# timescale/pgvectorscale

Measured on AMD Instinct MI355X. Metric: QPS at recall@10>=0.99, higher is better.
Workload: dtype u64 xor+popcount (SBQ) / f32 (rerank)

## Files before the change

pgvectorscale_amd/csrc/vs_batch.hip:

```cpp
#include <thread>
#include <cstdarg>
#include <cmath>
#include <algorithm>
#include <cstdlib>

#include <atomic>
#include <mutex>
#include <unordered_map>

#include "vs_internal.h"


static uint32_t knob_u32(const char* name, int tuned, uint32_t dflt) {
    const char* v = vs_opt_get(name);
    if (v && *v) return (uint32_t)strtoul(v, nullptr, 10);
    return tuned >= 0 ? (uint32_t)tuned : dflt;
}

static uint32_t gload_pct() { return std::min<uint32_t>(std::max<uint32_t>(env_u32("VS_F_GLOAD_PCT", 75), 25), 90); }

static Caps initial_caps(const vs_index* ix, uint32_t L, uint32_t M) {
    uint64_t visits = 2ull * L + M + 32;
    uint64_t pushes = visits * ix->d.num_neighbors;
    Caps c;
// ... 281 lines not shown
    return v && *v;
}
static uint32_t visited_want(uint32_t L) { return (uint32_t)std::min<uint64_t>((uint64_t)L + L / 2 + 32, 1u << 20); }

static int candidate_holds(vs_index* ix, const FastLaunch& base, const FastLaunch& cand, uint64_t num, uint64_t den, bool* holds,
                           const char* base_name = nullptr, const char* cand_name = nullptr, const char* tail = "") {
    uint32_t res_base = 0, res_cand = 0;
    VS_TRY(fast_resident_scans(ix, base, &res_base));
    VS_TRY(fast_resident_scans(ix, cand, &res_cand));
    if (base_name && env_u32("VS_WS_DEBUG", 0))
        fprintf(stderr, "[VS_WS_DEBUG] resident scans: %s %u, %s %u%s\n", base_name, res_base, cand_name, res_cand, tail);
    *holds = num * res_cand >= den * res_base;
    return VS_OK;
}

static int choose_table_bitmap(vs_index* ix, FastLaunch& f, uint32_t vmode, bool phase, bool* slot_eligible) {
    *slot_eligible = false;
    if (f.lh != 0 || f.vr || !vmode || phase || f.gcap > (1u << 16)) return VS_OK;
    f.vwords = (f.gcap + 127) / 128;
    if (vmode < 2 || f.rc || f.gcap % 32 != 0) return VS_OK;
    *slot_eligible = true;
    FastLaunch g = f;
    g.vwords = f.gcap / 32;
    g.vslot = 1;
    bool holds = false;
    VS_TRY(candidate_holds(ix, f, g, 1, 1, &holds));
    if (holds || env_u32("VS_F_SLOTMAP_FORCE", 0)) f = g;
    return VS_OK;
}

static int choose_tables16(vs_index* ix, FastLaunch& f, uint32_t vmode, bool slot_eligible, bool keyed, uint32_t* gregion) {
    if (vmode != 3 || !f.vwords || !slot_eligible || f.lh != 0) return VS_OK;
    FastLaunch g = f;
    g.gcap = std::max<uint32_t>(next_pow2_u32(f.gcap), 1024);
    if (!fast_tables16_geometry(ix, g)) return VS_OK;
    g.glimit = (uint32_t)((uint64_t)g.gcap * gload_pct() / 100) - 64u;
    char tail[48];
    snprintf(tail, sizeof tail, "; gcap %u -> %u", f.gcap, g.gcap);
    bool holds = false;
    VS_TRY(candidate_holds(ix, f, g, keyed ? 3 : 5, keyed ? 2 : 4, &holds, "4-byte tables", "16-bit tables", tail));
    if (holds || env_u32("VS_F_SLOTMAP_FORCE", 0)) {
        f = g;
        *gregion = g.gregion;
    }
    return VS_OK;
}

static int choose_heap_top(vs_index* ix, FastLaunch& f, Caps& caps, bool phase) {
    if (f.lh != 0 || f.vr || f.hl != 511 || f.hcap <= 511 || phase || opt_is_set("VS_F_HL")) return VS_OK;
    FastLaunch h = f;
    h.hl = 255;
    h.gstride = round_up_u32(h.hcap - h.hl + 2, 2);
    bool holds = false;
    VS_TRY(candidate_holds(ix, f, h, 10, 11, &holds, "heap top 511", "255"));
    if (holds) {
        f = h;
        caps.f_hl = h.hl;
        caps.f_gstride = h.gstride;
    }
    return VS_OK;
}

static int choose_visited_ring(vs_index* ix, FastLaunch& f, uint32_t L, bool phase) {
    if (f.lh != 0 || f.vr || f.minw == 7 || phase) return VS_OK;
    const uint32_t want_v = visited_want(L);
    const uint32_t lean_v = round_up_u32(std::max<uint32_t>(want_v + 2 * want_v / 5, 64), 64);
    if (opt_is_set("VS_F_VCAP") || lean_v >= f.vcap) return VS_OK;
// ... 136 lines not shown
static int bind_timeline_buffer(vs_index* ix, FastLaunch& f, std::string* path) {
    const char* const tl_opt = vs_opt_get("VS_TIMELINE");
    *path = tl_opt ? tl_opt : "";
    if (path->empty()) return VS_OK;
    SearchWorkspace& w = ix->ws;
    VS_TRY(devbuf_reserve(ix->ctx, w.timeline, (size_t)f.nq * 16));
    VS_HIP(hipMemsetAsync(w.timeline.p, 0, (size_t)f.nq * 16, ix->ctx->stream));
    f.timeline = (uint64_t*)w.timeline.p;
    return VS_OK;
}
static int dump_timeline(vs_index* ix, uint32_t nq, const std::string& path) {
    std::vector<uint64_t> tl((size_t)nq * 2);
    VS_HIP(hipMemcpyAsync(tl.data(), ix->ws.timeline.p, tl.size() * 8, hipMemcpyDeviceToHost, ix->ctx->stream));
    VS_HIP(hipStreamSynchronize(ix->ctx->stream));
    if (FILE* fp = fopen(path.c_str(), "wb")) {
        fwrite(tl.data(), 8, tl.size(), fp);
        fclose(fp);
    }
    return VS_OK;
}

static int dump_fast_status(vs_index* ix, const FastLaunch& f, double pool_frac) {
    vs_ctx* c = ix->ctx;
    SearchWorkspace& w = ix->ws;
    std::vector<uint32_t> stv(f.nq);
    VS_HIP(hipMemcpyAsync(stv.data(), w.status.p, (size_t)f.nq * 4, hipMemcpyDeviceToHost, c->stream));
    uint32_t ctr[2] = {0, 0};
    VS_HIP(hipMemcpyAsync(ctr, w.pool_ctr.p, 4, hipMemcpyDeviceToHost, c->stream));
    VS_HIP(hipStreamSynchronize(c->stream));
    uint32_t hist[16] = {0};
    for (uint32_t v : stv) hist[v & 15]++;
    fprintf(stderr, "[VS_DEBUG_STATUS] fast kernel: lh=%u gcap=%u vr=%u minw=%u bitmap_words=%u (per %s); pool claims=%u of %u;",
            f.lh, f.gcap, f.vr, f.minw, f.vwords, f.vslot == 2 ? "slot, 16-bit entries" : f.vslot ? "slot" : "bucket", ctr[0], fast_pool_slots(f.nq, pool_frac));
    for (int i = 0; i < 16; ++i)
        if (hist[i]) fprintf(stderr, " status[%d]=%u", i, hist[i]);
    fprintf(stderr, "\n");
    return VS_OK;
}

static int run_fast_attempts(vs_index* ix, const BatchPlan& bp, Caps& caps, const int16_t* d_qlabels, const uint32_t* d_qlabel_off) {
    vs_ctx* c = ix->ctx;
    SearchWorkspace& w = ix->ws;
    const uint8_t* const visible = (!bp.stream_only && bp.rescore > 0) ? ix->visible : nullptr;
    ix->last_ins_limit = caps.f_lh ? caps.f_lh - caps.f_lh / 8 - 64 : 0xFFFFFFFFu;
    FastPlan p;
    VS_TRY(plan_fast_launch(ix, bp, caps, d_qlabel_off != nullptr, visible != nullptr, &p));
    FastLaunch& f = p.f;
    VS_TRY(bind_fast_buffers(ix, p, d_qlabels, d_qlabel_off, visible));
    VS_TRY(bind_phase_buffer(ix, f));
    std::string tl_path;
    VS_TRY(bind_timeline_buffer(ix, f, &tl_path));
    hipEvent_t ev = prof_begin(c);
    VS_TRY(launch_search_fast(ix, f));
    prof_end(c, PK_SEARCH, ev);
    if (f.timeline) VS_TRY(dump_timeline(ix, bp.nq, tl_path));
    ix->last_fast = FastSig{f.vwords, f.minw, f.gcap, f.lh, f.vr, 1u};
    ix->last_info = vs_search_info{VS_SEARCH_FAST_SBQ, f.persist, (uint32_t)fast_lds_bytes(ix, f), f.hl, f.lh + f.gcap, f.vr ? 512u : f.vcap, {0, 0}};
    ix->last_info_valid = true;
    FastLaunch r;
    if (env_u32("VS_F_RETRY", 1) && second_attempt_of(ix, f, bp.nq, &r)) {
        VS_TRY(devbuf_reserve(c, w.heap_g4b, (size_t)r.pool_slots * r.gstride * 4));
        VS_TRY(devbuf_reserve(c, w.ghash4b, (size_t)r.pool_slots * r.gcap * 4));
        r.heap_g = (uint32_t*)w.heap_g4b.p;
        r.ghash = (uint32_t*)w.ghash4b.p;
        hipEvent_t ev2 = prof_begin(c);
        VS_TRY(launch_search_fast(ix, r));
// ... 470 lines not shown
```

pgvectorscale_amd/csrc/vs_internal.h:

```cpp
#pragma once
#include <hip/hip_runtime.h>

#include <cstdint>
#include <cstdio>
#include <cstring>
#include <string>
#include <atomic>
#include <mutex>
#include <vector>

#include "../../include/vsgpu.h"

#define VS_EMPTY 0xFFFFFFFFu

void vs_set_error(const char* fmt, ...);
const char* vs_opt_get(const char* name);

#define VS_HIP(expr)                                                                                   \
    do {                                                                                               \
        hipError_t _e = (expr);                                                                        \
        if (_e != hipSuccess) {                                                                        \
            vs_set_error("%s failed: %s (%s:%d)", #expr, hipGetErrorString(_e), __FILE__, __LINE__);   \
            return (_e == hipErrorOutOfMemory) ? VS_ERR_OOM : VS_ERR_HIP;                              \
        }                                                                                              \
    } while (0)

#define VS_REQUIRE(cond, ...)         \
    do {                              \
        if (!(cond)) {                \
            vs_set_error(__VA_ARGS__);\
            return VS_ERR_INVALID;    \
        }                             \
    } while (0)

#define VS_REQUIRE_OOM(cond, ...)     \
    do {                              \
        if (!(cond)) {                \
            vs_set_error(__VA_ARGS__);\
            return VS_ERR_OOM;        \
        }                             \
    } while (0)

#define VS_TRY(expr)            \
    do {                        \
// ... 236 lines not shown
    uint32_t* out_ids;
    uint32_t* out_ham;
    uint32_t* out_cnt;
    uint32_t* stats;
    uint32_t* status;
    uint32_t only_failed = 0;
    uint32_t* pool_counter = nullptr;
    uint32_t pool_slots = 0;
    uint32_t* fb_flag = nullptr;
    const uint8_t* visible = nullptr;
    uint32_t* resume = nullptr;
    uint32_t resume_stride = 0;
    uint32_t* row_stats = nullptr;
};
enum { RS_INIT = 0, RS_HLEN, RS_HMAX, RS_VLEN, RS_GLEV, RS_NINS_L, RS_NINS_G, RS_NINS_TOP, RS_VISITS, RS_CAND, RS_DQ, RS_READS,
       RS_NEXT, RS_INVIS, RS_STATUS, RS_EMITTED, RS_HDR = 16 };
size_t search_resume_words(const SearchLaunch& s);
struct FastLaunch {
    uint32_t nq, L, M;
    uint32_t hl;
    uint32_t hcap;
    uint32_t gstride;
    uint32_t lh;
    uint32_t gcap;
    uint32_t glimit = 0;
    uint32_t sb;
    uint32_t vr;
    uint32_t vcap;
    uint32_t minw;
    uint32_t rc = 0;
    uint32_t persist = 0;
    uint32_t vwords = 0;
    uint32_t vslot = 0;
    uint32_t qd = 0, qk = 0, ocap = 0, gregion = 0;
    uint32_t build = 0;
    uint32_t flags = 0;
    uint32_t only_failed = 0;
    uint32_t* fb_flag = nullptr;
    const uint8_t* visible = nullptr;
    const uint64_t* qcodes;
    const int16_t* qlabels;
    const uint32_t* qlabel_off;
    uint32_t* heap_g;
    uint32_t* ghash;
    uint32_t* pool_counter;
    uint32_t pool_slots;
    uint32_t* out_ids;
    uint32_t* out_ham;
    uint32_t* out_cnt;
    uint32_t* stats;
    uint32_t* status;
    uint64_t* phase = nullptr;
    uint32_t* scan_counter = nullptr;
    uint64_t* timeline = nullptr;
    uint32_t* resume = nullptr;
    uint32_t resume_stride = 0;
    uint32_t* row_stats = nullptr;
};
enum { RSF_INIT = 0, RSF_HLEN, RSF_VHEAD, RSF_VLEN, RSF_NINS_G, RSF_N_OVF, RSF_HMAX, RSF_VISITS, RSF_CAND, RSF_POPS, RSF_INVIS, RSF_STATUS,
       RSF_NEXT, RSF_ENDED, RSF_HDR = 16 };
size_t fast_resume_words(const FastLaunch& s);
enum {
    FAST_FULL_VARIANT = 8,
};
size_t fast_lds_bytes(const vs_index* idx, const FastLaunch& s);
static inline bool fast_tables16_geometry(const vs_index* idx, FastLaunch& f) {
    uint32_t qd = 1, lb = 0;
    while ((1ull << qd) < (uint64_t)(idx->d.n > 2 ? idx->d.n : 2)) qd++;
    while ((1u << lb) < (f.gcap >> 3)) lb++;
    if (qd < lb + 3) qd = lb + 3;
    f.qd = qd;
    f.qk = qd - lb;
    const uint32_t o = round_up_u32(f.gcap / 16, 32);
    f.ocap = o > 256 ? o : 256;
    f.vwords = (f.gcap + f.ocap) / 32;
    f.vslot = 2;
    f.gregion = (f.gcap >> 1) + f.ocap;
    f.sb = 0;
    while ((1ull << f.sb) < (uint64_t)f.gcap + f.ocap) f.sb++;
    const uint64_t nbits = (uint64_t)idx->d.dim_index * idx->d.bits;
    return f.qk <= 16 && f.qd <= 32 && nbits < (1ull << (32 - f.sb));
}
int launch_search_fast(vs_index* idx, const FastLaunch& s);
int fast_resident_scans(vs_index* idx, const FastLaunch& s, uint32_t* out);
struct PlainLaunch {
    uint32_t nq, L, M;
    uint32_t hl;
    uint32_t hcap;
    uint32_t vcap;
    uint32_t slots;
    uint32_t ins_limit;
    uint32_t lds_table;
    uint32_t persist;
    uint32_t resident = 0;
    const uint8_t* visible = nullptr;
    uint64_t* heap_g = nullptr;
    uint32_t* table_g = nullptr;
    uint32_t* scan_counter = nullptr;
    uint32_t* out_ids = nullptr;
    uint32_t* out_ham = nullptr;
    uint32_t* out_cnt = nullptr;
    uint32_t* stats = nullptr;
    uint32_t* status = nullptr;
    const float* q_prepared = nullptr;
    uint32_t* resume = nullptr;
    uint32_t resume_stride = 0;
    uint32_t* row_stats = nullptr;
};
enum { RSP_INIT = 0, RSP_HLEN, RSP_HMAX, RSP_VHEAD, RSP_VLEN, RSP_NINS, RSP_VISITS, RSP_CAND, RSP_DQ, RSP_READS, RSP_NEXT, RSP_INVIS,
       RSP_STATUS, RSP_EMITTED, RSP_ENDED, RSP_HDR = 16 };
static_assert((int)RSP_HDR == (int)RS_HDR && (int)RSP_HDR == (int)RSF_HDR, "a pool clears one header size at amrescan, whichever kernel continues its scans");
static const uint32_t PLAIN_LDS_TABLE_MAX = 1024;
size_t plain_lds_bytes(const vs_index* idx, const PlainLaunch& s);
size_t plain_resume_words(const PlainLaunch& s);
// ... 53 lines not shown
```

pgvectorscale_amd/csrc/vs_scanpool.cpp:

```cpp
#include <algorithm>
#include <chrono>
#include <cstring>
#include <vector>

#include "vs_internal.h"

namespace {

struct Slot {
    bool active = false, null_query = false, keys = false, exhausted = false, failed = false, masked = false;
    std::vector<int16_t> labels;
    uint32_t rows = 0;
    uint32_t handed = 0;
    uint32_t calls_after_end = 0;
    std::vector<uint32_t> row_stats;
    uint32_t final_counters[ST_N] = {0};
    uint32_t launches = 0;
};

}

struct vs_scan_pool {
    vs_index* ix = nullptr;
    uint32_t cap = 0, L = 0, rescore = 0, S = 0, kmax = 0, rows_cap = 0, mmax = 0;
// ... 87 lines not shown
    VS_REQUIRE(kmax >= 1 && kmax <= 4096, "vs_scanpool_create: rows per fetch outside [1,4096]");
    *out = nullptr;
    vs_ctx* c = ix->ctx;
    VS_HIP(hipSetDevice(c->device));
    vs_scan_pool* p = new vs_scan_pool();
    p->ix = ix;
    p->cap = capacity;
    p->L = L;
    p->rescore = rescore;
    p->S = (ix->d.storage_type == VS_STORAGE_PLAIN && ix->d.dim_index == ix->d.dim_full) ? 0u : rescore;
    p->kmax = kmax;
    p->rows_cap = std::max<uint32_t>(rows_cap ? rows_cap : 4096, p->S + kmax);
    p->mmax = p->S + kmax;
    const uint64_t visits = 2ull * L + p->rows_cap + 32;
    const uint64_t pushes = visits * ix->d.num_neighbors;
    p->hl = pool_env_u32("VS_HL", 1024);
    p->lh = 0;
    p->g0 = pool_env_u32("VS_G0", 4096);
    p->hcap = (uint32_t)std::min<uint64_t>(std::max<uint64_t>(pushes, p->hl), 1u << 24);
    p->vcap = (uint32_t)std::min<uint64_t>(2ull * L + 256, 1u << 20);
    p->hashcap = std::max<uint32_t>(next_pow2_u32(std::min<uint64_t>(2ull * pushes, 1u << 26)), p->g0);
    SearchLaunch probe{};
    probe.hl = p->hl;
    probe.lh = p->lh;
    probe.vcap = p->vcap;
    p->rw = (uint32_t)search_resume_words(probe);
    if (ix->d.storage_type != VS_STORAGE_PLAIN && pool_env_u32("VS_POOL_FAST", 1) && ix->d.n > 0) {
        FastLaunch f{};
        f.hl = 511;
        f.hcap = (uint32_t)std::min<uint64_t>(std::max<uint64_t>(pushes, f.hl), 1u << 22);
        f.gstride = round_up_u32(f.hcap - f.hl + 2, 2);
        f.vcap = round_up_u32(std::max<uint32_t>(2u * (uint32_t)std::min<uint64_t>((uint64_t)L + L / 2 + 32, 1u << 16), 64), 64);
        f.minw = 1;
        f.gcap = std::max<uint32_t>(next_pow2_u32(std::min<uint64_t>(pushes * 4 / 3 + 256, 1u << 22)), 1024);
        f.glimit = (uint32_t)((uint64_t)f.gcap * 3 / 4) - 64u;
        const uint32_t nch = (ix->code_stride + 7) / 8;
        if (fast_tables16_geometry(ix, f) && nch <= 6 && fast_lds_bytes(ix, f) <= POOL_LDS_BUDGET) {
            p->fast = true;
            p->fl = f;
            p->rw = (uint32_t)fast_resume_words(f);
        }
    }
    if (plan_plain_pool(ix, L, pushes, &p->pl)) {
        p->plain_fast = true;
        p->rw = (uint32_t)plain_resume_words(p->pl);
    }
    p->slots.resize(capacity);
    const size_t G = capacity;
    auto all = [&]() -> int {
        VS_TRY(devbuf_reserve(c, p->raw_q, G * ix->d.dim_full * 4));
        VS_TRY(devbuf_reserve(c, p->q_full, G * ix->vec_stride * 4));
        VS_TRY(devbuf_reserve(c, p->qcodes, G * ix->code_stride * 8 + 16));
        if (ix->d.storage_type == VS_STORAGE_PLAIN && ix->d.dim_index < ix->d.dim_full) VS_TRY(devbuf_reserve(c, p->q_index, G * ix->vec_stride * 4));
        VS_TRY(devbuf_reserve(c, p->qlabel_off, (G + 1) * 4));
        VS_TRY(devbuf_reserve(c, p->qlabels, 64));
        if (p->fast) {
            VS_TRY(devbuf_reserve(c, p->heap_g, std::max<size_t>(G * (size_t)p->fl.gstride * 4, 16)));
            VS_TRY(devbuf_reserve(c, p->hash, G * (size_t)p->fl.gregion * 4));
        } else if (p->plain_fast) {
            VS_TRY(devbuf_reserve(c, p->heap_g, std::max<size_t>(G * (size_t)(p->pl.hcap - p->pl.hl) * 8, 16)));
            VS_TRY(devbuf_reserve(c, p->hash, std::max<size_t>(p->pl.lds_table ? 0 : G * (size_t)p->pl.slots * 4, 16)));
        } else {
            VS_TRY(devbuf_reserve(c, p->heap_g, std::max<size_t>(G * (size_t)(p->hcap > p->hl ? p->hcap - p->hl : 0) * 8, 16)));
            VS_TRY(devbuf_reserve(c, p->hash, G * (size_t)p->hashcap * 4));
        }
        VS_TRY(devbuf_reserve(c, p->state, G * (size_t)p->rw * 4));
        VS_TRY(devbuf_reserve(c, p->cnt, G * 4));
// ... 531 lines not shown
```

pgvectorscale_amd/csrc/vs_search_fast.hip:

```cpp
#ifndef VS_FAST_TU
#define VS_FAST_TU 0
#endif
#include <cstdlib>

#include "vs_device.h"

#define MAX_QLABELS 64
#define VS_Q16_A 0x9E3779B1u
#define VS_Q16_B 0x85EBCA6Bu
#define VS_Q16_AI 0x0E8B2F51u
#define VS_Q16_BI 0xA5CB9243u
static_assert((uint32_t)(VS_Q16_A * VS_Q16_AI) == 1u && (uint32_t)(VS_Q16_B * VS_Q16_BI) == 1u, "inverse multipliers");
#define ARB_SLOTS 128

struct FastArgs {
    const uint64_t* codes;
    const uint32_t* nbrs;
    const uint64_t* tids;
    const uint32_t* label_off;
    const int16_t* label_val;
    const uint64_t* label_mask;
    const uint8_t* label_bit;
    const uint64_t* nbr_mask;
    const int16_t* ls_labels;
    const uint32_t* ls_nodes;
    uint32_t code_stride, nbr_stride, R, n, n_ls, default_start;
    FastLaunch s;
};

__device__ __forceinline__ void wave_sync() {
    __builtin_amdgcn_fence(__ATOMIC_RELEASE, "wavefront");
    __builtin_amdgcn_wave_barrier();
    __builtin_amdgcn_fence(__ATOMIC_ACQUIRE, "wavefront");
}
typedef __attribute__((address_space(1))) uint32_t glb_u32;
typedef __attribute__((address_space(1))) uint64_t glb_u64;
typedef __attribute__((address_space(3))) uint32_t lds_u32;
typedef __attribute__((address_space(1))) uint16_t glb_u16;
__device__ __forceinline__ uint32_t gload32(const uint32_t* p) { return *(const glb_u32*)p; }
__device__ __forceinline__ void gstore32(uint32_t* p, uint32_t v) { *(glb_u32*)p = v; }
__device__ __forceinline__ uint64_t gload64u(const uint64_t* p) { return *(const glb_u64*)p; }
__device__ __forceinline__ uint32_t gload16(const uint16_t* p) { return (uint32_t)*(const glb_u16*)p; }
__device__ __forceinline__ void gstore16(uint16_t* p, uint32_t v) { *(glb_u16*)p = (uint16_t)v; }
__device__ __forceinline__ uint32_t lload32(const uint32_t* p) { return *(const lds_u32*)p; }
__device__ __forceinline__ void lstore32(uint32_t* p, uint32_t v) { *(lds_u32*)p = v; }
// ... 671 lines not shown
            const uint64_t now = __builtin_readcyclecounter();
            ph[k] += now - tmark;
            tmark = now;
        }
    };

    uint32_t* ghash = s.ghash;
    const uint32_t gbuckets = s.gcap >> 2;
    uint32_t nins_g = 0;
    bool g_open = false, region = false;
    auto claim_region = [&]() -> bool {
        if (region) return true;
        if (s.persist || RS) {
            region = true;
            ghash = s.ghash + (size_t)slot * (VG == 3 ? s.gregion : s.gcap);
            return true;
        }
        uint32_t pslot = 0;
        if (lane == 0) pslot = atomicAdd(s.pool_counter, 1u);
        pslot = rfl(pslot);
        if (pslot >= s.pool_slots) {
            status |= OVF_POOL;
            return false;
        }
        region = true;
        ghash = s.ghash + (size_t)pslot * (VG == 3 ? s.gregion : s.gcap);
        if (onlyfv) heap.g = s.heap_g + (size_t)pslot * s.gstride;
        return true;
    };
    auto hash_home = [&](uint32_t nid) -> uint32_t { return (uint32_t)(((uint64_t)hash_u32(nid) * lhv) >> 32); };
    auto g_empty = [&](uint32_t v) -> bool { return v == VS_EMPTY; };
    const uint32_t qdm = in_vgpr(VG == 3 ? (s.qd >= 32 ? 0xFFFFFFFFu : (1u << s.qd) - 1u) : 0u);
    const uint32_t qxs = in_vgpr((s.qd + 1u) >> 1);
    const uint32_t qk_v = in_vgpr(s.qk), rmask_v = in_vgpr((1u << s.qk) - 1u);
    const uint32_t ovf_lim_v = in_vgpr(s.ocap - s.ocap / 4);
    auto q_fwd = [&](uint32_t id) -> uint32_t {
        uint32_t x = (id * VS_Q16_A) & qdm;
        x ^= x >> qxs;
        x = (x * VS_Q16_B) & qdm;
        x ^= x >> qxs;
        return x;
    };
    auto q_inv = [&](uint32_t x) -> uint32_t {
        x ^= x >> qxs;
        x = (x * VS_Q16_BI) & qdm;
        x ^= x >> qxs;
        return (x * VS_Q16_AI) & qdm;
    };
    auto node_load = [&](uint32_t handle) -> uint32_t {
        if (VG == 3) {
            if (handle < s.gcap) return gload16(reinterpret_cast<const uint16_t*>(ghash) + handle);
            return gload32(ghash + (s.gcap >> 1) + (handle - s.gcap));
        }
        if (handle < lhv) return lload32(lhash + handle);
        return gload32(ghash + (handle - lhv));
    };
    auto node_of = [&](uint32_t handle, uint32_t raw) -> uint32_t {
        if (VG == 3 && handle < s.gcap) return rfl(q_inv(((handle >> 3) << qk_v) | raw));
        return raw;
    };
    auto finish_insert = [&](uint32_t nid, bool act, uint32_t slot, uint32_t old, uint32_t& slot_out) -> bool {
        bool fresh = false;
        if (act) {
            for (;;) {
                if (old == VS_EMPTY) { fresh = true; break; }
                if (old == nid) break;
                slot = slot + 1 == lhv ? 0 : slot + 1;
                old = atomicCAS(&lhash[slot], VS_EMPTY, nid);
            }
            slot_out = slot;
        }
        nins += (uint32_t)__popcll(__ballot(fresh));
        return fresh;
    };
    const bool gmode = lhv == 0;
    auto ghash_home = [&](uint32_t nid) -> uint32_t {
        return (uint32_t)(((uint64_t)hash_u32(nid ^ 0x5bd1e995u) * gbuckets) >> 32) << 2;
    };
    auto bucket_load = [&](uint32_t b0) -> uint4 { return *reinterpret_cast<const uint4*>(ghash + b0); };
    auto bucket_fetch = [&](uint32_t b0, bool& virgin) -> uint4 {
        if (VG) {
            const uint32_t b = b0 >> 2;
            virgin = ((vmap[b >> 5] >> (b & 31u)) & 1u) == 0;
            if (virgin) return make_uint4(VS_EMPTY, VS_EMPTY, VS_EMPTY, VS_EMPTY);
        }
        return bucket_load(b0);
    };
    auto global_insert = [&](uint32_t nid, bool act, uint32_t b0, uint4 v, bool virgin, uint32_t& slot_out) -> bool {
        bool fresh = false, pend = act;
        for (;;) {
            wave_sync();
// ... 59 lines not shown
                t = slot_run(pos);
                if (t) v = *reinterpret_cast<const uint4*>(ghash + (pos & ~3u));
            }
            pre_t = 0;
            if (pend && t == 0) {
                const uint32_t bit = 1u << (pos & 31u);
                if ((atomicOr(&vmap[pos >> 5], bit) & bit) == 0) {
                    ghash[pos] = nid;
                    slot_out = lhv + pos;
                    fresh = true;
                    pend = false;
                } else {
                    pos = pos + 1 == s.gcap ? 0u : pos + 1;
                }
            } else if (pend) {
                const uint32_t hit = ((v.x == nid ? 1u : 0u) | (v.y == nid ? 2u : 0u) | (v.z == nid ? 4u : 0u) | (v.w == nid ? 8u : 0u)) &
                                     (((1u << t) - 1u) << (pos & 3u));
                if (hit) {
                    slot_out = lhv + (pos & ~3u) + (uint32_t)__builtin_ctz(hit);
                    pend = false;
                } else {
                    pos += t;
                    if (pos == s.gcap) pos = 0;
                }
            }
            wave_sync();
            if (!__ballot(pend)) break;
        }
        nins_g += (uint32_t)__popcll(__ballot(fresh));
        return fresh;
    };
    auto b16_occ = [&](uint32_t hb) -> uint32_t { return (vmap[hb >> 2] >> ((hb & 3u) << 3)) & 0xFFu; };
    auto b16_run = [&](uint32_t x) -> uint32_t {
        const uint32_t occ = b16_occ(x >> qk_v);
        const uint32_t rot = ((occ | (occ << 8)) >> (x & 7u)) & 0xFFu;
        return (uint32_t)__builtin_ctz(~rot);
    };
    auto b16_load = [&](uint32_t x) -> uint4 { return *reinterpret_cast<const uint4*>(ghash + ((size_t)(x >> qk_v) << 2)); };
    uint32_t n_ovf = 0;
    auto ovf_insert = [&](uint32_t nid, bool act, uint32_t& slot_out) -> bool {
        uint32_t* const ot = ghash + (s.gcap >> 1);
        uint32_t* const om = vmap + (s.gcap >> 5);
        auto orun = [&](uint32_t pos) -> uint32_t {
            const uint32_t g = pos & ~3u;
            const uint32_t rel = ((om[g >> 5] >> (g & 31u)) & 0xFu) >> (pos & 3u);
            return (uint32_t)__builtin_ctz(~rel);
        };
        bool fresh = false, pend = act;
        uint32_t pos = (uint32_t)(((uint64_t)hash_u32(nid ^ 0x5bd1e995u) * s.ocap) >> 32);
        for (;;) {
            wave_sync();
            uint32_t t = 0;
            uint4 v = make_uint4(0, 0, 0, 0);
            if (pend) {
                t = orun(pos);
                if (t) v = *reinterpret_cast<const uint4*>(ot + (pos & ~3u));
            }
            if (pend && t == 0) {
                const uint32_t bit = 1u << (pos & 31u);
                if ((atomicOr(&om[pos >> 5], bit) & bit) == 0) {
                    ot[pos] = nid;
                    slot_out = lhv + s.gcap + pos;
                    fresh = true;
                    pend = false;
                } else {
                    pos = pos + 1 == s.ocap ? 0u : pos + 1;
                }
            } else if (pend) {
                const uint32_t hit = ((v.x == nid ? 1u : 0u) | (v.y == nid ? 2u : 0u) | (v.z == nid ? 4u : 0u) | (v.w == nid ? 8u : 0u)) &
                                     (((1u << t) - 1u) << (pos & 3u));
                if (hit) {
                    slot_out = lhv + s.gcap + (pos & ~3u) + (uint32_t)__builtin_ctz(hit);
                    pend = false;
                } else {
                    pos += t;
                    if (pos == s.ocap) pos = 0;
                }
            }
            wave_sync();
            if (!__ballot(pend)) break;
        }
        n_ovf += (uint32_t)__popcll(__ballot(fresh));
        return fresh;
    };
    auto b16_insert = [&](uint32_t nid, bool act, uint32_t x, uint4 v, uint32_t pre_t, bool have_pre, uint32_t& slot_out) -> bool {
        uint32_t t = pre_t;
        if (!have_pre) {
            wave_sync();
            t = act ? b16_run(x) : 0u;
            v = make_uint4(0, 0, 0, 0);
            if (t) v = b16_load(x);
        }
        const uint32_t hb = x >> qk_v, r = x & rmask_v, pref = x & 7u;
        const uint32_t rr = r | (r << 16);
        uint32_t one = 0x00010001u;
        asm volatile("" : "+v"(one));
        const uint32_t z = pk_min_u16(v.x ^ rr, one) | (pk_min_u16(v.y ^ rr, one) << 2) | (pk_min_u16(v.z ^ rr, one) << 4) | (pk_min_u16(v.w ^ rr, one) << 6);
        const uint32_t m = ~(z | (z >> 15)) & 0xFFu;
        uint32_t rm = ((1u << t) - 1u) << pref;
        rm = (rm | (rm >> 8)) & 0xFFu;
        const uint32_t hit = act ? (m & rm) : 0u;
        if (hit) slot_out = lhv + (hb << 3) + (uint32_t)__builtin_ctz(hit);
        uint64_t pendm = __ballot(act && hit == 0), freshm = 0, ovfm = 0;
        uint32_t t2 = t;
        while (pendm) {
            wave_sync();
            const uint32_t idx = (hb << 3) + ((pref + t2) & 7u);
            const uint32_t bit = 1u << (idx & 31u);
            const bool mine = lane_of(pendm);
            uint32_t old = 0xFFFFFFFFu;
            if (mine && t2 < 8u) old = atomicOr(&vmap[idx >> 5], bit);
            const bool won = (old & bit) == 0;
            if (won) {
                gstore16(reinterpret_cast<uint16_t*>(ghash) + idx, r);
                slot_out = lhv + idx;
            }
            const uint64_t wonm = __ballot(won), fullm = __ballot(mine && t2 >= 8u);
            freshm |= wonm;
            ovfm |= fullm;
            pendm &= ~(wonm | fullm);
            wave_sync();
            if (!pendm) break;
            const uint32_t occ = b16_occ(hb);
            t2 = (uint32_t)__builtin_ctz(~(((occ | (occ << 8)) >> pref) & 0xFFu));
        }
        bool fresh = lane_of(freshm);
// ... 433 lines not shown
            rs[RSF_NEXT] = st_next;
            rs[RSF_ENDED] = ended ? 1u : 0u;
        }
    }
    if (status == 0) {
        for (uint32_t i = emitted + lane; i < s.M; i += WAVE) {
            s.out_ids[(size_t)q * s.M + i] = VS_INVALID_NODE;
            s.out_ham[(size_t)q * s.M + i] = 0xFFFFFFFFu;
        }
    }
    if (lane == 0) {
        if (onlyfv && s.fb_flag) s.fb_flag[q] = 1;
        s.status[q] = status;
        s.out_cnt[q] = status ? 0 : emitted;
        if (status == 0) {
            uint32_t* st = s.stats + (size_t)q * ST_N;
            st[ST_VISITS] = st_visits;
            st[ST_CAND] = st_cand;
            st[ST_DQ] = st_cand;
            st[ST_READS] = st_pops + st_visits + nins + nins_g;
            st[ST_NEXT] = st_next;
            st[ST_GSPILL] = hmax;
            st[ST_INVIS] = st_invis;
            st[7] = nins + nins_g;
        }
        if (TIMING && s.phase) {
            lap(6);
            for (int k = 0; k < 8; ++k) s.phase[(size_t)q * 8 + k] = ph[k];
        }
        if (s.timeline) s.timeline[2 * (size_t)q + 1] = wall_clock64();
    }
}

template <int NCH, int VR, bool TIMING, int MINW, bool BUILD, bool FULL = true, int VG = 0, int OPT = 0>
__global__ __launch_bounds__(WAVE, MINW) void k_search_fast(FastArgs a) {
    for (uint32_t it = 0;; ++it) {
        uint32_t q = blockIdx.x;
        if (a.s.persist) {
            if (threadIdx.x == 0) q = atomicAdd(a.s.scan_counter, 1u);
            q = rfl(q);
        } else if (it) {
            return;
        }
        if (q >= a.s.nq) return;
        fast_scan<NCH, VR, TIMING, MINW, BUILD, FULL, VG, OPT>(a, q, blockIdx.x);
        wave_sync();
    }
}

#if VS_FAST_TU == 0
size_t fast_resume_words(const FastLaunch& s) { return RSF_HDR + ((size_t)(s.hl + 1) + 2 * (size_t)s.vcap + s.vwords + 3) / 4 * 4; }

size_t fast_lds_bytes(const vs_index* idx, const FastLaunch& s) {
    const size_t nch = (idx->code_stride + 7) / 8;
    const size_t qcopy = nch > 6 ? (size_t)idx->code_stride * 8 : (s.minw >= 6 && !s.build && !s.phase ? nch * 64 : 0);
    const bool lean = s.minw == 7 && s.vslot == 2 && nch == 3 && !s.build && !s.phase;
    const bool plain = !s.qlabel_off && !s.visible && !(s.flags & FAST_FULL_VARIANT);
    size_t b = (size_t)(s.hl + 1) * 4 + (size_t)s.lh * 4 + (lean ? 2 : 3) * 64 * 4 + (s.vslot ? 0 : ARB_SLOTS * 4) + (s.vr ? 0 : (size_t)s.vcap * 8) +
               (lean && plain ? 0 : MAX_QLABELS * 2) + qcopy + (size_t)s.rc * 4 + (size_t)s.vwords * 4 + (lean ? 16 : 32);
    return (b + 15) / 16 * 16;
}

#endif

template <int NCH, int VR, bool TIMING, int MINW, bool BUILD, bool FULL = true, int VG = 0, int OPT = 0>
static int launch_fast_tt(vs_index* idx, const FastArgs& a, size_t lds, uint32_t* resident) {
    static DeviceOnce attr_set;
    const int attr_dev = idx->ctx->device;
// ... 8 lines not shown
        *resident = (uint32_t)std::max(per_cu, 1) * (uint32_t)idx->ctx->prop.multiProcessorCount;
        return VS_OK;
    }
    const uint32_t grid = a.s.persist ? std::min<uint32_t>(a.s.persist, a.s.nq) : a.s.nq;
    hipLaunchKernelGGL((k_search_fast<NCH, VR, TIMING, MINW, BUILD, FULL, VG, OPT>), dim3(grid), dim3(WAVE), lds, idx->ctx->stream, a);
    VS_HIP(hipGetLastError());
    return VS_OK;
}

int launch_fast_plain6(vs_index* idx, const FastArgs& a, size_t lds, uint32_t* res, bool std_geom);
int launch_fast_keys6(vs_index* idx, const FastArgs& a, size_t lds, uint32_t* res, bool std_geom);
#if VS_FAST_TU == 1
int launch_fast_plain6(vs_index* idx, const FastArgs& a, size_t lds, uint32_t* res, bool std_geom) {
    if (std_geom) return launch_fast_tt<3, 0, false, 6, false, false, 3, OPT_XW | OPT_R1 | OPT_NS64>(idx, a, lds, res);
    return launch_fast_tt<3, 0, false, 6, false, false, 3>(idx, a, lds, res);
}
#elif VS_FAST_TU == 2
int launch_fast_keys6(vs_index* idx, const FastArgs& a, size_t lds, uint32_t* res, bool std_geom) {
    if (std_geom) return launch_fast_tt<3, 0, false, 6, false, true, 3, OPT_XW | OPT_R1 | OPT_NS64>(idx, a, lds, res);
    return launch_fast_tt<3, 0, false, 6, false, true, 3>(idx, a, lds, res);
}
#else
template <int NCH>
static int launch_fast_t(vs_index* idx, const FastArgs& a, size_t lds, uint32_t* res) {
    if (a.s.build) {
        VS_REQUIRE(a.s.vr == 0 && !a.s.phase, "build-mode search uses the LDS-ring visited list");
        return launch_fast_tt<NCH, 0, false, 1, true>(idx, a, lds, res);
    }
    if (a.s.phase) {
        VS_REQUIRE(NCH == 3, "VS_PHASE diagnostics are built for 17..24-word codes only");
        if (a.s.vr == 8) return launch_fast_tt<3, 8, true, 1, false>(idx, a, lds, res);
        return launch_fast_tt<3, 0, true, 1, false>(idx, a, lds, res);
    }
    if (a.s.resume) {
        VS_REQUIRE(a.s.vwords && a.s.vslot == 2 && !a.s.persist && a.s.vr == 0 && a.s.lh == 0 && a.s.rc == 0 && !a.s.only_failed && a.s.pool_slots >= a.s.nq,
                   "fast search: resumable scans run the 16-bit tables with one region per slot");
        return launch_fast_tt<NCH, 0, false, 1, false, true, 3, OPT_RS>(idx, a, lds, res);
    }
    if (a.s.vwords && a.s.vslot == 2) {
        VS_REQUIRE(a.s.vr == 0 && a.s.lh == 0 && a.s.rc == 0 && a.s.gcap >= 256 && (a.s.gcap & (a.s.gcap - 1)) == 0 && a.s.ocap % 32 == 0 && a.s.ocap >= 64 &&
                       (uint64_t)a.s.vwords * 32 >= (uint64_t)a.s.gcap + a.s.ocap && a.s.qk >= 3 && a.s.qk <= 16 && a.s.qd <= 32 &&
                       (1ull << a.s.qd) == ((uint64_t)(a.s.gcap >> 3) << a.s.qk) && (a.s.qd >= 32 || a.n <= (1ull << a.s.qd)) &&
                       a.s.gregion >= (a.s.gcap >> 1) + a.s.ocap,
                   "fast search: bad geometry of the 16-bit dedup table");
        const bool plain = !a.s.qlabel_off && !a.s.visible && !(a.s.flags & FAST_FULL_VARIANT);
        const bool std_geom = a.code_stride == 24 && a.R <= WAVE && a.nbr_stride == 64;
        if (NCH == 3 && a.s.minw == 6 && plain) return launch_fast_plain6(idx, a, lds, res, std_geom);
        if (NCH == 3 && a.s.minw == 6) return launch_fast_keys6(idx, a, lds, res, std_geom);
        if (NCH == 3 && a.s.minw == 7 && plain && std_geom) return launch_fast_tt<3, 0, false, 7, false, false, 3, OPT_XW | OPT_R1 | OPT_NS64>(idx, a, lds, res);
        if (NCH == 3 && a.s.minw == 7 && plain) return launch_fast_tt<3, 0, false, 7, false, false, 3>(idx, a, lds, res);
        if (NCH == 3 && a.s.minw == 7) return launch_fast_tt<3, 0, false, 7, false, true, 3>(idx, a, lds, res);
        return launch_fast_tt<NCH, 0, false, 1, false, true, 3>(idx, a, lds, res);
    }
    if (a.s.vwords && a.s.vslot) {
        VS_REQUIRE(a.s.vr == 0 && a.s.lh == 0 && (uint64_t)a.s.vwords * 32 >= a.s.gcap && a.s.rc == 0,
                   "fast search: the slot bitmap needs the table-less regime and one bit per slot");
        const bool plain = !a.s.qlabel_off && !a.s.visible && !(a.s.flags & FAST_FULL_VARIANT);
        if (NCH == 3 && a.s.minw == 6 && plain) return launch_fast_tt<3, 0, false, 6, false, false, 2>(idx, a, lds, res);
        if (NCH == 3 && a.s.minw == 6) return launch_fast_tt<3, 0, false, 6, false, true, 2>(idx, a, lds, res);
        return launch_fast_tt<NCH, 0, false, 1, false, true, 2>(idx, a, lds, res);
    }
    if (a.s.vwords) {
        VS_REQUIRE(a.s.vr == 0 && a.s.lh == 0 && (uint64_t)a.s.vwords * 128 >= a.s.gcap,
                   "fast search: the written-bucket bitmap needs the table-less regime and one bit per bucket");
        const bool plain = !a.s.qlabel_off && !a.s.visible && !(a.s.flags & FAST_FULL_VARIANT);
        if (NCH == 3 && a.s.minw == 6 && plain) return launch_fast_tt<3, 0, false, 6, false, false, 1>(idx, a, lds, res);
        if (NCH == 3 && a.s.minw == 6) return launch_fast_tt<3, 0, false, 6, false, true, 1>(idx, a, lds, res);
        if (NCH == 3 && a.s.minw == 5 && plain) return launch_fast_tt<3, 0, false, 5, false, false, 1>(idx, a, lds, res);
        if (NCH == 3 && a.s.minw == 5) return launch_fast_tt<3, 0, false, 5, false, true, 1>(idx, a, lds, res);
        return launch_fast_tt<NCH, 0, false, 1, false, true, 1>(idx, a, lds, res);
    }
    if (a.s.vr == 8) {
        if (NCH == 3) {
            if (a.s.minw == 4) return launch_fast_tt<3, 8, false, 4, false>(idx, a, lds, res);
            if (a.s.minw == 5) return launch_fast_tt<3, 8, false, 5, false>(idx, a, lds, res);
            if (a.s.minw == 6) return launch_fast_tt<3, 8, false, 6, false>(idx, a, lds, res);
        }
// ... 69 lines not shown
```

Baseline: 4.327 million.

## Size 16-bit dedup tables to multiples of 256 with magic-division bucket mapping

```diff
diff --git a/pgvectorscale_amd/csrc/vs_batch.hip b/pgvectorscale_amd/csrc/vs_batch.hip
--- a/pgvectorscale_amd/csrc/vs_batch.hip
+++ b/pgvectorscale_amd/csrc/vs_batch.hip
@@ -337,7 +337,7 @@
 static int choose_tables16(vs_index* ix, FastLaunch& f, uint32_t vmode, bool slot_eligible, bool keyed, uint32_t* gregion) {
     if (vmode != 3 || !f.vwords || !slot_eligible || f.lh != 0) return VS_OK;
     FastLaunch g = f;
-    g.gcap = std::max<uint32_t>(next_pow2_u32(f.gcap), 1024);
+    g.gcap = std::max<uint32_t>(round_up_u32(f.gcap, 256), 1024);
     if (!fast_tables16_geometry(ix, g)) return VS_OK;
     g.glimit = (uint32_t)((uint64_t)g.gcap * gload_pct() / 100) - 64u;
     char tail[48];
@@ -540,6 +540,9 @@
     for (uint32_t v : stv) hist[v & 15]++;
     fprintf(stderr, "[VS_DEBUG_STATUS] fast kernel: lh=%u gcap=%u vr=%u minw=%u bitmap_words=%u (per %s); pool claims=%u of %u;",
             f.lh, f.gcap, f.vr, f.minw, f.vwords, f.vslot == 2 ? "slot, 16-bit entries" : f.vslot ? "slot" : "bucket", ctr[0], fast_pool_slots(f.nq, pool_frac));
+    if (f.vslot == 2)
+        fprintf(stderr, " q16: %u buckets x %u entries (qd=%u qm=%#x qs=%u) ocap=%u table_bytes=%u;", f.gcap >> 3, f.qe, f.qd, f.qm, f.qs, f.ocap, f.gregion * 4);
+    fprintf(stderr, " hl=%u vcap=%u lds_bytes=%zu resident=%u;", f.hl, f.vr ? 512u : f.vcap, fast_lds_bytes(ix, f), f.persist);
     for (int i = 0; i < 16; ++i)
         if (hist[i]) fprintf(stderr, " status[%d]=%u", i, hist[i]);
     fprintf(stderr, "\n");
diff --git a/pgvectorscale_amd/csrc/vs_internal.h b/pgvectorscale_amd/csrc/vs_internal.h
--- a/pgvectorscale_amd/csrc/vs_internal.h
+++ b/pgvectorscale_amd/csrc/vs_internal.h
@@ -10,6 +10,7 @@
 #include <vector>
 
 #include "../../include/vsgpu.h"
+#include "vs_q16.h"
 
 #define VS_EMPTY 0xFFFFFFFFu
 
@@ -312,7 +313,7 @@
     uint32_t persist = 0;
     uint32_t vwords = 0;
     uint32_t vslot = 0;
-    uint32_t qd = 0, qk = 0, ocap = 0, gregion = 0;
+    uint32_t qd = 0, qe = 0, qm = 0, qs = 0, ocap = 0, gregion = 0;
     uint32_t build = 0;
     uint32_t flags = 0;
     uint32_t only_failed = 0;
@@ -345,21 +346,19 @@
 };
 size_t fast_lds_bytes(const vs_index* idx, const FastLaunch& s);
 static inline bool fast_tables16_geometry(const vs_index* idx, FastLaunch& f) {
-    uint32_t qd = 1, lb = 0;
-    while ((1ull << qd) < (uint64_t)(idx->d.n > 2 ? idx->d.n : 2)) qd++;
-    while ((1u << lb) < (f.gcap >> 3)) lb++;
-    if (qd < lb + 3) qd = lb + 3;
-    f.qd = qd;
-    f.qk = qd - lb;
-    const uint32_t o = round_up_u32(f.gcap / 16, 32);
-    f.ocap = o > 256 ? o : 256;
-    f.vwords = (f.gcap + f.ocap) / 32;
+    Q16Geometry g;
+    const bool ok = q16_geometry(idx->d.n, f.gcap, &g);
+    f.qd = g.qd;
+    f.qe = g.qe;
+    f.qm = g.qm;
+    f.qs = g.qs;
+    f.ocap = g.ocap;
+    f.vwords = g.vwords;
     f.vslot = 2;
-    f.gregion = (f.gcap >> 1) + f.ocap;
-    f.sb = 0;
-    while ((1ull << f.sb) < (uint64_t)f.gcap + f.ocap) f.sb++;
+    f.gregion = g.gregion;
+    f.sb = g.sb;
     const uint64_t nbits = (uint64_t)idx->d.dim_index * idx->d.bits;
-    return f.qk <= 16 && f.qd <= 32 && nbits < (1ull << (32 - f.sb));
+    return ok && nbits < (1ull << (32 - f.sb));
 }
 int launch_search_fast(vs_index* idx, const FastLaunch& s);
 int fast_resident_scans(vs_index* idx, const FastLaunch& s, uint32_t* out);
diff --git a/pgvectorscale_amd/csrc/vs_q16.h b/pgvectorscale_amd/csrc/vs_q16.h
--- /dev/null
+++ b/pgvectorscale_amd/csrc/vs_q16.h
@@ -0,0 +1,86 @@
+#pragma once
+#include <cstdint>
+
+#if defined(__HIPCC__) || defined(__host__)
+#define VS_Q16_HD __host__ __device__ static inline
+#else
+#define VS_Q16_HD static inline
+#endif
+
+#define VS_Q16_A 0x9E3779B1u
+#define VS_Q16_B 0x85EBCA6Bu
+#define VS_Q16_AI 0x0E8B2F51u
+#define VS_Q16_BI 0xA5CB9243u
+static_assert((uint32_t)(VS_Q16_A * VS_Q16_AI) == 1u && (uint32_t)(VS_Q16_B * VS_Q16_BI) == 1u, "inverse multipliers");
+
+VS_Q16_HD uint32_t q16_mask(uint32_t qd) { return qd >= 32 ? 0xFFFFFFFFu : (1u << qd) - 1u; }
+VS_Q16_HD uint32_t q16_xshift(uint32_t qd) { return (qd + 1u) >> 1; }
+VS_Q16_HD uint32_t q16_fwd(uint32_t id, uint32_t qdm, uint32_t qxs) {
+    uint32_t x = (id * VS_Q16_A) & qdm;
+    x ^= x >> qxs;
+    x = (x * VS_Q16_B) & qdm;
+    x ^= x >> qxs;
+    return x;
+}
+VS_Q16_HD uint32_t q16_inv(uint32_t x, uint32_t qdm, uint32_t qxs) {
+    x ^= x >> qxs;
+    x = (x * VS_Q16_BI) & qdm;
+    x ^= x >> qxs;
+    return (x * VS_Q16_AI) & qdm;
+}
+
+VS_Q16_HD uint32_t q16_mul24(uint32_t a, uint32_t b) {
+#if defined(__HIP_DEVICE_COMPILE__)
+    return __umul24(a, b);
+#else
+    return a * b;
+#endif
+}
+VS_Q16_HD uint32_t q16_bucket(uint32_t x, uint32_t qm, uint32_t qs) {
+#if defined(__HIP_DEVICE_COMPILE__)
+    return __umulhi(x, qm) >> (qs & 31u);
+#else
+    return (uint32_t)(((uint64_t)x * qm) >> 32) >> (qs & 31u);
+#endif
+}
+VS_Q16_HD uint32_t q16_entry(uint32_t x, uint32_t bucket, uint32_t qe) { return x - q16_mul24(bucket, qe); }
+VS_Q16_HD uint32_t q16_join(uint32_t bucket, uint32_t entry, uint32_t qe) { return q16_mul24(bucket, qe) + entry; }
+
+struct Q16Geometry {
+    uint32_t qd;
+    uint32_t qe;
+    uint32_t qm, qs;
+    uint32_t ocap;
+    uint32_t vwords;
+    uint32_t gregion;
+    uint32_t sb;
+};
+static inline bool q16_geometry(uint64_t n, uint32_t gcap, Q16Geometry* g) {
+    *g = Q16Geometry{};
+    if (gcap < 256 || gcap % 256 != 0 || gcap > (1u << 26)) return false;
+    const uint32_t nb = gcap >> 3;
+    uint32_t qd = 1, lb = 0;
+    while (qd < 40 && (1ull << qd) < (n > 2 ? n : 2)) qd++;
+    while ((1u << lb) < nb) lb++;
+    if (qd < lb + 3) qd = lb + 3;
+    g->qd = qd;
+    const uint32_t o = (gcap / 16 + 127) / 128 * 128;
+    g->ocap = o > 256 ? o : 256;
+    g->vwords = (gcap + g->ocap) / 32;
+    g->gregion = (gcap >> 1) + g->ocap;
+    g->sb = 0;
+    while ((1ull << g->sb) < (uint64_t)gcap + g->ocap) g->sb++;
+    g->qe = g->qm = g->qs = 0;
+    if (qd > 32) return false;
+    const uint64_t qe = ((1ull << qd) + nb - 1) / nb;
+    if (qe > 65536) return false;
+    uint32_t qs = 0;
+    while ((2ull << qs) < qe) qs++;
+    const uint64_t two = 1ull << (32 + qs);
+    const uint64_t qm = (two + qe - 1) / qe;
+    if (qm >> 32 || ((qm * qe - two) << qd) > two) return false;
+    g->qe = (uint32_t)qe;
+    g->qm = (uint32_t)qm;
+    g->qs = qs;
+    return true;
+}
diff --git a/pgvectorscale_amd/csrc/vs_scanpool.cpp b/pgvectorscale_amd/csrc/vs_scanpool.cpp
--- a/pgvectorscale_amd/csrc/vs_scanpool.cpp
+++ b/pgvectorscale_amd/csrc/vs_scanpool.cpp
@@ -143,7 +143,7 @@
         f.gstride = round_up_u32(f.hcap - f.hl + 2, 2);
         f.vcap = round_up_u32(std::max<uint32_t>(2u * (uint32_t)std::min<uint64_t>((uint64_t)L + L / 2 + 32, 1u << 16), 64), 64);
         f.minw = 1;
-        f.gcap = std::max<uint32_t>(next_pow2_u32(std::min<uint64_t>(pushes * 4 / 3 + 256, 1u << 22)), 1024);
+        f.gcap = std::max<uint32_t>(round_up_u32((uint32_t)std::min<uint64_t>(pushes * 4 / 3 + 256, 1u << 22), 256), 1024);
         f.glimit = (uint32_t)((uint64_t)f.gcap * 3 / 4) - 64u;
         const uint32_t nch = (ix->code_stride + 7) / 8;
         if (fast_tables16_geometry(ix, f) && nch <= 6 && fast_lds_bytes(ix, f) <= POOL_LDS_BUDGET) {
diff --git a/pgvectorscale_amd/csrc/vs_search_fast.hip b/pgvectorscale_amd/csrc/vs_search_fast.hip
--- a/pgvectorscale_amd/csrc/vs_search_fast.hip
+++ b/pgvectorscale_amd/csrc/vs_search_fast.hip
@@ -6,11 +6,6 @@
 #include "vs_device.h"
 
 #define MAX_QLABELS 64
-#define VS_Q16_A 0x9E3779B1u
-#define VS_Q16_B 0x85EBCA6Bu
-#define VS_Q16_AI 0x0E8B2F51u
-#define VS_Q16_BI 0xA5CB9243u
-static_assert((uint32_t)(VS_Q16_A * VS_Q16_AI) == 1u && (uint32_t)(VS_Q16_B * VS_Q16_BI) == 1u, "inverse multipliers");
 #define ARB_SLOTS 128
 
 struct FastArgs {
@@ -748,21 +743,11 @@
     auto g_empty = [&](uint32_t v) -> bool { return v == VS_EMPTY; };
     const uint32_t qdm = in_vgpr(VG == 3 ? (s.qd >= 32 ? 0xFFFFFFFFu : (1u << s.qd) - 1u) : 0u);
     const uint32_t qxs = in_vgpr((s.qd + 1u) >> 1);
-    const uint32_t qk_v = in_vgpr(s.qk), rmask_v = in_vgpr((1u << s.qk) - 1u);
+    const uint32_t qm_v = in_vgpr(s.qm), qc_v = in_vgpr((s.qe << 5) | s.qs);
     const uint32_t ovf_lim_v = in_vgpr(s.ocap - s.ocap / 4);
-    auto q_fwd = [&](uint32_t id) -> uint32_t {
-        uint32_t x = (id * VS_Q16_A) & qdm;
-        x ^= x >> qxs;
-        x = (x * VS_Q16_B) & qdm;
-        x ^= x >> qxs;
-        return x;
-    };
-    auto q_inv = [&](uint32_t x) -> uint32_t {
-        x ^= x >> qxs;
-        x = (x * VS_Q16_BI) & qdm;
-        x ^= x >> qxs;
-        return (x * VS_Q16_AI) & qdm;
-    };
+    auto q_fwd = [&](uint32_t id) -> uint32_t { return q16_fwd(id, qdm, qxs); };
+    auto q_inv = [&](uint32_t x) -> uint32_t { return q16_inv(x, qdm, qxs); };
+    auto q_bucket = [&](uint32_t x) -> uint32_t { return q16_bucket(x, qm_v, qc_v); };
     auto node_load = [&](uint32_t handle) -> uint32_t {
         if (VG == 3) {
             if (handle < s.gcap) return gload16(reinterpret_cast<const uint16_t*>(ghash) + handle);
@@ -772,7 +757,7 @@
         return gload32(ghash + (handle - lhv));
     };
     auto node_of = [&](uint32_t handle, uint32_t raw) -> uint32_t {
-        if (VG == 3 && handle < s.gcap) return rfl(q_inv(((handle >> 3) << qk_v) | raw));
+        if (VG == 3 && handle < s.gcap) return rfl(q_inv(q16_join(handle >> 3, raw, qc_v >> 5)));
         return raw;
     };
     auto finish_insert = [&](uint32_t nid, bool act, uint32_t slot, uint32_t old, uint32_t& slot_out) -> bool {
@@ -898,11 +883,11 @@
     };
     auto b16_occ = [&](uint32_t hb) -> uint32_t { return (vmap[hb >> 2] >> ((hb & 3u) << 3)) & 0xFFu; };
     auto b16_run = [&](uint32_t x) -> uint32_t {
-        const uint32_t occ = b16_occ(x >> qk_v);
+        const uint32_t occ = b16_occ(q_bucket(x));
         const uint32_t rot = ((occ | (occ << 8)) >> (x & 7u)) & 0xFFu;
         return (uint32_t)__builtin_ctz(~rot);
     };
-    auto b16_load = [&](uint32_t x) -> uint4 { return *reinterpret_cast<const uint4*>(ghash + ((size_t)(x >> qk_v) << 2)); };
+    auto b16_load = [&](uint32_t x) -> uint4 { return *reinterpret_cast<const uint4*>(ghash + ((size_t)q_bucket(x) << 2)); };
     uint32_t n_ovf = 0;
     auto ovf_insert = [&](uint32_t nid, bool act, uint32_t& slot_out) -> bool {
         uint32_t* const ot = ghash + (s.gcap >> 1);
@@ -957,7 +942,7 @@
             v = make_uint4(0, 0, 0, 0);
             if (t) v = b16_load(x);
         }
-        const uint32_t hb = x >> qk_v, r = x & rmask_v, pref = x & 7u;
+        const uint32_t hb = q_bucket(x), r = q16_entry(x, hb, qc_v >> 5), pref = x & 7u;
         const uint32_t rr = r | (r << 16);
         uint32_t one = 0x00010001u;
         asm volatile("" : "+v"(one));
@@ -1457,8 +1442,12 @@
     }
 }
 
+#define FAST_WAVES(MINW, FULL, VG, OPT) (((MINW) == 6 && !(FULL) && (VG) == 3 && (OPT) == (OPT_XW | OPT_R1 | OPT_NS64)) ? 7 : (MINW))
 template <int NCH, int VR, bool TIMING, int MINW, bool BUILD, bool FULL = true, int VG = 0, int OPT = 0>
-__global__ __launch_bounds__(WAVE, MINW) void k_search_fast(FastArgs a) {
+__global__ __launch_bounds__(WAVE, FAST_WAVES(MINW, FULL, VG, OPT)) void k_search_fast(FastArgs a) {
+#if defined(__HIP_DEVICE_COMPILE__)
+    if (FAST_WAVES(MINW, FULL, VG, OPT) != MINW) asm volatile("" ::: "v71");
+#endif
     for (uint32_t it = 0;; ++it) {
         uint32_t q = blockIdx.x;
         if (a.s.persist) {
@@ -1533,17 +1522,23 @@
         if (a.s.vr == 8) return launch_fast_tt<3, 8, true, 1, false>(idx, a, lds, res);
         return launch_fast_tt<3, 0, true, 1, false>(idx, a, lds, res);
     }
+    if (a.s.vwords && a.s.vslot == 2) {
+        VS_REQUIRE(a.s.vr == 0 && a.s.lh == 0 && a.s.rc == 0 && a.s.gcap >= 256 && a.s.gcap % 256 == 0 && a.s.ocap % 32 == 0 && a.s.ocap >= 64 &&
+                       (uint64_t)a.s.vwords * 32 >= (uint64_t)a.s.gcap + a.s.ocap && a.s.qd <= 32 && (a.s.qd >= 32 || a.n <= (1ull << a.s.qd)) &&
+                       a.s.gregion >= (a.s.gcap >> 1) + a.s.ocap,
+                   "fast search: bad geometry of the 16-bit dedup table");
+        Q16Geometry qg;
+        VS_REQUIRE(q16_geometry(a.n, a.s.gcap, &qg) && qg.qd == a.s.qd && qg.qe == a.s.qe && qg.qm == a.s.qm && qg.qs == a.s.qs && a.s.qe >= 8 &&
+                       a.s.qe <= 65536 && (uint64_t)a.s.qe * (a.s.gcap >> 3) >= (1ull << a.s.qd) && (a.s.gcap >> 3) < (1u << 24),
+                   "fast search: the 16-bit dedup table's bucket / entry constants do not belong to this index and table size");
+    }
     if (a.s.resume) {
         VS_REQUIRE(a.s.vwords && a.s.vslot == 2 && !a.s.persist && a.s.vr == 0 && a.s.lh == 0 && a.s.rc == 0 && !a.s.only_failed && a.s.pool_slots >= a.s.nq,
                    "fast search: resumable scans run the 16-bit tables with one region per slot");
+        VS_REQUIRE(a.s.vwords % 4 == 0 && (a.s.hl + 1) % 4 == 0, "fast search: a resumable scan's LDS image must be whole 16-byte words");
         return launch_fast_tt<NCH, 0, false, 1, false, true, 3, OPT_RS>(idx, a, lds, res);
     }
     if (a.s.vwords && a.s.vslot == 2) {
-        VS_REQUIRE(a.s.vr == 0 && a.s.lh == 0 && a.s.rc == 0 && a.s.gcap >= 256 && (a.s.gcap & (a.s.gcap - 1)) == 0 && a.s.ocap % 32 == 0 && a.s.ocap >= 64 &&
-                       (uint64_t)a.s.vwords * 32 >= (uint64_t)a.s.gcap + a.s.ocap && a.s.qk >= 3 && a.s.qk <= 16 && a.s.qd <= 32 &&
-                       (1ull << a.s.qd) == ((uint64_t)(a.s.gcap >> 3) << a.s.qk) && (a.s.qd >= 32 || a.n <= (1ull << a.s.qd)) &&
-                       a.s.gregion >= (a.s.gcap >> 1) + a.s.ocap,
-                   "fast search: bad geometry of the 16-bit dedup table");
         const bool plain = !a.s.qlabel_off && !a.s.visible && !(a.s.flags & FAST_FULL_VARIANT);
         const bool std_geom = a.code_stride == 24 && a.R <= WAVE && a.nbr_stride == 64;
         if (NCH == 3 && a.s.minw == 6 && plain) return launch_fast_plain6(idx, a, lds, res, std_geom);
```

New measurement: 4.448 million (median of 6 runs). 2.8% higher.
